# hukenovs/blackman_harris_win

Measured on AMD Instinct MI355X. Metric: window Gsamples/s (BH-7, N=2^26, 32-bit) + fraction of HBM-write roofline, higher is better.
Workload: dtype int64

## Files before the change

### blackman_harris_win_amd/csrc/bhw_build.hip

```cpp
#include "bhw_device.h"

namespace {

template <typename T>
__global__ __launch_bounds__(kBlock) void k_table_build(BhwCordicCfg cfg, uint32_t entries, void *__restrict__ table)
{
    __shared__ T lut_s[32];
    stage_lut<T>(cfg, lut_s);
    const uint32_t u = blockIdx.x * kBlock + threadIdx.x;
    if (u >= entries) return;
    T x, y;
    cordic_q1<T>(lut_s, (T)cfg.x0, (T)((T)u << cfg.z_shl), (int)cfg.n_iter, x, y);
    const int32_t c = (int32_t)(x >> cfg.out_shr), sn = (int32_t)(y >> cfg.out_shr);
    const int2 head = make_int2(__builtin_amdgcn_readfirstlane(c), __builtin_amdgcn_readfirstlane(sn));
    const int4 rec = cfg.tab_dlog > kPackLog ? reinterpret_cast<const int4 *>(cfg.tab_coarse)[u >> fmt_cell_log(cfg.tab_dlog)] : make_int4(0, 0, 0, 0);
    tab_store(table, u, cfg.phi_width - 2 - cfg.z_shr, cfg.tab_split, cfg.tab_dlog, const_cast<void *>(cfg.tab_coarse), c, sn, head, rec,
              cfg.tab_check);
}


template <int NITER, int FMT>
__global__ __launch_bounds__(kBuildThreads) void k_table_build_shared(BhwBuildPlan plan, void *__restrict__ table)
{
    __shared__ int64_t gx[kGroupsPerWg];
    __shared__ int64_t gy[kGroupsPerWg];
    __shared__ int32_t gz[kGroupsPerWg];
    __shared__ int32_t gk[kGroupsPerWg];
    __shared__ uint32_t lut_s[32];
    if (threadIdx.x < 32) lut_s[threadIdx.x] = plan.lut[threadIdx.x];
    __syncthreads();

    constexpr int n_iter = NITER;
    const uint32_t s = plan.z_shl;
    const uint32_t gpw = plan.groups_per_wg;
    const uint32_t group0 = blockIdx.x * gpw;
    const uint32_t n_groups = plan.entries >> 6;

    if (threadIdx.x < gpw) {
        const uint32_t g = group0 + threadIdx.x;
        const uint32_t u_first = g << 6;
        int64_t x = plan.x0, y = plan.x0;
        int32_t zf = (int32_t)((u_first << s) - lut_s[0]);
        const uint32_t span = 63u << s;
        int k = 1;
        bool live = g < n_groups;
        constexpr int kmax = n_iter < kPrefixMax ? n_iter : kPrefixMax;
#pragma unroll
        for (int kk = 1; kk < kmax; ++kk) {
            if (live) {
                const int32_t zl = (int32_t)((uint32_t)zf + span);
                if ((zf < 0) != (zl < 0)) {
                    live = false;
                } else {
                    rot_step(x, y, zf, kk, plan.lut[kk]);
                    k = kk + 1;
                }
            }
        }
        gx[threadIdx.x] = x;
        gy[threadIdx.x] = y;
        gz[threadIdx.x] = zf;
        gk[threadIdx.x] = k;
    }
    __syncthreads();

    const uint32_t wave = __builtin_amdgcn_readfirstlane(threadIdx.x >> 6), lane = threadIdx.x & 63u;
    uint32_t idx_a = lane, idx_m = 64u;
    if (plan.tab_split) {
        const uint32_t e = 1u << plan.log2_entries;
        if (lane & 1u)      { idx_a = (e >> 1) + (lane >> 1); idx_m = 32u; }
        else if (lane & 2u) { idx_a = (e >> 2) + (lane >> 2); idx_m = 16u; }
        else                { idx_a = lane >> 2;              idx_m = 16u; }
    }
    for (uint32_t gi = wave; gi < gpw; gi += kBuildThreads / 64) {
        const uint32_t g = __builtin_amdgcn_readfirstlane(group0 + gi);
        if (g >= n_groups) break;
        int64_t x = gx[gi], y = gy[gi];
        int32_t z = (int32_t)((uint32_t)gz[gi] + (lane << s));
        const int k0 = __builtin_amdgcn_readfirstlane(gk[gi]);
#pragma unroll
        for (int k = 1; k < NITER; ++k) {
            if (k >= kPrefixMax || k >= k0) rot_step(x, y, z, k, plan.lut[k]);
        }
        const int32_t c = (int32_t)(x >> plan.out_shr), sn = (int32_t)(y >> plan.out_shr);
        const int2 head = make_int2(__builtin_amdgcn_readfirstlane(c), __builtin_amdgcn_readfirstlane(sn));
        const uint32_t idx = idx_a + g * idx_m;
        if constexpr (FMT == 4) {
            const uint32_t u = (g << 6) + lane, nmask = 4u * plan.entries - 1u;
            int32_t *d_sin = reinterpret_cast<int32_t *>(table), *d_cos = reinterpret_cast<int32_t *>(const_cast<void *>(plan.tab_coarse));
#pragma unroll
            for (uint32_t q = 0; q < 4u; ++q) {
                int32_t oc, os;
                quadrant_map(q, c, sn, plan.pad0, oc, os);
                const uint32_t i = (q * plan.entries + u - plan.pad) & nmask;
                if (d_sin) d_sin[i] = os;
                if (d_cos) d_cos[i] = oc;
            }
        } else if constexpr (FMT == 0) {
            reinterpret_cast<int2 *>(table)[idx] = make_int2(c, sn);
        } else {
            static_assert(FMT == 1, "k_table_build_shared builds plain and delta16 tables (and the sin / cos sweep) only");
            const int32_t dc = c - head.x, ds = sn - head.y;
            if (plan.check_flag && !(fits_bits(dc, 16) && fits_bits(ds, 16))) atomicOr(plan.check_flag, 1u);
            reinterpret_cast<uint32_t *>(table)[idx] = ((uint32_t)dc & 0xFFFFu) | ((uint32_t)ds << 16);
            if (lane == 0u) reinterpret_cast<int2 *>(const_cast<void *>(plan.tab_coarse))[g] = head;
        }
    }
}

constexpr int kMirrorTail = 6;
constexpr int mirror_gpw(int threads) { return threads / 4; }
constexpr int mirror_heads_max(int threads) { return mirror_gpw(threads) / 2 + 8; }
constexpr int mirror_heads_pad(int threads) { return (mirror_heads_max(threads) + 63) / 64 * 64; }
constexpr int kTailZ = 256;

constexpr int kTailRows = 65;
struct TailD { int8_t v[kTailRows * 64 + 16]; };
constexpr TailD make_tail_d()
{
    TailD t{};
    for (int p = 0; p < 64; ++p)
        for (int v = 0; v < kTailRows; ++v) {
            int d = 0;
            for (int j = 0; j < kMirrorTail; ++j) d += ((p >> j) & 1) ? -(v >> j) : (v >> j);
            t.v[v * 64 + p] = (int8_t)d;
        }
    return t;
}
__device__ const TailD kTailD = make_tail_d();

template <int K, bool ZERO>
__device__ __forceinline__ void rot_narrow(uint32_t &x, uint32_t &y, int32_t &z, uint32_t &zacc, uint32_t lutk)
{
    uint32_t a, b;
    if constexpr (ZERO) {
        asm volatile("v_lshrrev_b32 %[a], %[k], %[y]\n\t"
                     "v_lshrrev_b32 %[b], %[k], %[x]\n\t"
                     "v_min_u32 %[za], %[za], %[z]\n\t"
                     "v_cmpx_gt_i32 vcc, 0, %[z]\n\t"
                     "v_add_u32 %[x], %[x], %[a]\n\t"
                     "v_sub_u32 %[y], %[y], %[b]\n\t"
                     "v_add_u32 %[z], %[z], %[l]\n\t"
                     "s_not_b64 exec, exec\n\t"
                     "v_sub_u32 %[x], %[x], %[a]\n\t"
                     "v_add_u32 %[y], %[y], %[b]\n\t"
                     "v_sub_u32 %[z], %[z], %[l]\n\t"
                     "s_mov_b64 exec, -1"
                     : [x] "+v"(x), [y] "+v"(y), [z] "+v"(z), [za] "+v"(zacc), [a] "=&v"(a), [b] "=&v"(b)
                     : [l] "s"(lutk), [k] "n"(K)
                     : "vcc", "scc");
    } else {
        asm volatile("v_lshrrev_b32 %[a], %[k], %[y]\n\t"
                     "v_lshrrev_b32 %[b], %[k], %[x]\n\t"
                     "v_cmpx_gt_i32 vcc, 0, %[z]\n\t"
                     "v_add_u32 %[x], %[x], %[a]\n\t"
                     "v_sub_u32 %[y], %[y], %[b]\n\t"
                     "v_add_u32 %[z], %[z], %[l]\n\t"
                     "s_not_b64 exec, exec\n\t"
                     "v_sub_u32 %[x], %[x], %[a]\n\t"
                     "v_add_u32 %[y], %[y], %[b]\n\t"
                     "v_sub_u32 %[z], %[z], %[l]\n\t"
                     "s_mov_b64 exec, -1"
                     : [x] "+v"(x), [y] "+v"(y), [z] "+v"(z), [a] "=&v"(a), [b] "=&v"(b)
                     : [l] "s"(lutk), [k] "n"(K)
                     : "vcc", "scc");
    }
}

template <int KA, int NITER>
__device__ __forceinline__ void rot_narrow_block(uint32_t &x, uint32_t &y, int32_t &z, uint32_t &zacc, const uint32_t *lut, int e, uint32_t hi)
{
    uint32_t a, b;
#define BHW_ROT_I(lbl, i, HI_ADD)                                                                                       \
    #lbl ":\n\t"                                                                                                        \
    "v_lshrrev_b32 %[a], %[k" #i "], %[y]\n\t"                                                                          \
    "v_lshrrev_b32 %[b], %[k" #i "], %[x]\n\t"                                                                          \
    HI_ADD                                                                                                             \
    "v_min_u32 %[za], %[za], %[z]\n\t"                                                                                  \
    "v_cmpx_gt_i32 vcc, 0, %[z]\n\t"                                                                                    \
    "v_add_u32 %[x], %[x], %[a]\n\t"                                                                                    \
    "v_sub_u32 %[y], %[y], %[b]\n\t"                                                                                    \
    "v_add_u32 %[z], %[z], %[l" #i "]\n\t"                                                                              \
    "s_not_b64 exec, exec\n\t"                                                                                          \
    "v_sub_u32 %[x], %[x], %[a]\n\t"                                                                                    \
    "v_add_u32 %[y], %[y], %[b]\n\t"                                                                                    \
    "v_sub_u32 %[z], %[z], %[l" #i "]\n\t"                                                                              \
    "s_mov_b64 exec, -1\n"
#define BHW_ROT_PLAIN(i) BHW_ROT_I(i, i, "")
#define BHW_ROT_HI(i) BHW_ROT_I(2##i, i, "v_add_u32 %[b], %[c" #i "], %[b]\n\t")
#define BHW_ROT_DISPATCH(P)                                                                                            \
                 "s_cmp_lt_i32 %[e], 1\n\ts_cbranch_scc1 " #P "0f\n\t"                                                 \
                 "s_cmp_eq_u32 %[e], 1\n\ts_cbranch_scc1 " #P "1f\n\t"                                                 \
                 "s_cmp_eq_u32 %[e], 2\n\ts_cbranch_scc1 " #P "2f\n\t"                                                 \
                 "s_cmp_eq_u32 %[e], 3\n\ts_cbranch_scc1 " #P "3f\n\t"                                                 \
                 "s_cmp_eq_u32 %[e], 4\n\ts_cbranch_scc1 " #P "4f\n\t"                                                 \
                 "s_cmp_eq_u32 %[e], 5\n\ts_cbranch_scc1 " #P "5f\n\t"                                                 \
                 "s_cmp_eq_u32 %[e], 6\n\ts_cbranch_scc1 " #P "6f\n\t"                                                 \
                 "s_cmp_eq_u32 %[e], 7\n\ts_cbranch_scc1 " #P "7f\n\t"                                                 \
                 "s_cmp_eq_u32 %[e], 8\n\ts_cbranch_scc1 " #P "8f\n\t"                                                 \
                 "s_cmp_eq_u32 %[e], 9\n\ts_cbranch_scc1 " #P "9f\n\t"
    constexpr int S = NITER - 1 - KA;
    static_assert(S >= 9 && S <= 30, "bias shifts");
    asm volatile("s_cmp_lg_u32 %[hi], 0\n\ts_cbranch_scc1 100f\n\t"
                 BHW_ROT_DISPATCH()
                 "s_branch 10f\n"
                 BHW_ROT_PLAIN(0) BHW_ROT_PLAIN(1) BHW_ROT_PLAIN(2) BHW_ROT_PLAIN(3) BHW_ROT_PLAIN(4) BHW_ROT_PLAIN(5) BHW_ROT_PLAIN(6) BHW_ROT_PLAIN(7)
                 BHW_ROT_PLAIN(8) BHW_ROT_PLAIN(9)
                 "10:\n\ts_branch 200f\n"
                 "100:\n\t"
                 BHW_ROT_DISPATCH(2)
                 "s_branch 200f\n"
                 BHW_ROT_HI(0) BHW_ROT_HI(1) BHW_ROT_HI(2) BHW_ROT_HI(3) BHW_ROT_HI(4) BHW_ROT_HI(5) BHW_ROT_HI(6) BHW_ROT_HI(7) BHW_ROT_HI(8) BHW_ROT_HI(9)
                 "200:"
                 : [x] "+v"(x), [y] "+v"(y), [z] "+v"(z), [za] "+v"(zacc), [a] "=&v"(a), [b] "=&v"(b)
                 : [e] "s"(e), [hi] "s"(hi), [l0] "s"(lut[KA]), [l1] "s"(lut[KA + 1]), [l2] "s"(lut[KA + 2]), [l3] "s"(lut[KA + 3]), [l4] "s"(lut[KA + 4]),
                   [l5] "s"(lut[KA + 5]), [l6] "s"(lut[KA + 6]), [l7] "s"(lut[KA + 7]), [l8] "s"(lut[KA + 8]), [l9] "s"(lut[KA + 9]),
                   [k0] "n"(KA), [k1] "n"(KA + 1), [k2] "n"(KA + 2), [k3] "n"(KA + 3), [k4] "n"(KA + 4), [k5] "n"(KA + 5), [k6] "n"(KA + 6),
                   [k7] "n"(KA + 7), [k8] "n"(KA + 8), [k9] "n"(KA + 9),
                   [c0] "n"(1 << S), [c1] "n"(1 << (S - 1)), [c2] "n"(1 << (S - 2)), [c3] "n"(1 << (S - 3)), [c4] "n"(1 << (S - 4)),
                   [c5] "n"(1 << (S - 5)), [c6] "n"(1 << (S - 6)), [c7] "n"(1 << (S - 7)), [c8] "n"(1 << (S - 8)), [c9] "n"(1 << (S - 9))
                 : "vcc", "scc");
#undef BHW_ROT_I
#undef BHW_ROT_PLAIN
#undef BHW_ROT_HI
#undef BHW_ROT_DISPATCH
}

#ifdef BHW_BUILD_STAMPS
__device__ unsigned long long *g_build_stamps = nullptr;
#define BHW_STAMP(i) do { if (g_build_stamps && (threadIdx.x & 63u) == 0u) atomicMax(&g_build_stamps[blockIdx.x * 16u + (i)], (unsigned long long)wall_clock64()); } while (0)
#define BHW_STAMP_MIN(i) do { if (g_build_stamps && threadIdx.x == 0u) g_build_stamps[blockIdx.x * 16u + (i)] = (unsigned long long)wall_clock64(); } while (0)
#else
#define BHW_STAMP(i) do { } while (0)
#define BHW_STAMP_MIN(i) do { } while (0)
#endif

template <int BYTES>
__device__ __forceinline__ void table_store(void *__restrict__ table, uint32_t idx, uint32_t v)
{
    if constexpr (BYTES == 1) asm volatile("global_store_byte %0, %1, %2 sc1" :: "v"(idx), "v"(v), "s"(table) : "memory");
    else asm volatile("global_store_short %0, %1, %2 sc1" :: "v"(idx << 1), "v"(v), "s"(table) : "memory");
}

template <int NITER, int FMT, int THREADS>
__global__ __launch_bounds__(THREADS) __attribute__((amdgpu_waves_per_eu(8, 8))) void k_table_build_mirror(BhwBuildPlan plan, void *__restrict__ table)
{
    BHW_STAMP_MIN(0);
#ifdef BHW_BUILD_STAMPS
    if (g_build_stamps && threadIdx.x == 0u) {
        uint32_t hw, xcc;
        asm volatile("s_getreg_b32 %0, hwreg(HW_REG_HW_ID)\n\ts_getreg_b32 %1, hwreg(HW_REG_XCC_ID)" : "=s"(hw), "=s"(xcc));
        g_build_stamps[blockIdx.x * 16u + 6u] = hw;
        g_build_stamps[blockIdx.x * 16u + 7u] = xcc;
    }
#endif
    static_assert(FMT == 2 || FMT == 3 || FMT == 5, "residual / nibble entries");
    static_assert(NITER >= 21 && NITER <= 32, "narrow state: 32-bit words");
    static_assert(THREADS == 256 || THREADS == 1024, "workgroup shapes");
    constexpr uint32_t gpw = mirror_gpw(THREADS);
    constexpr uint32_t kHeads = mirror_heads_max(THREADS), kHeadsPad = mirror_heads_pad(THREADS);
    static_assert(gpw + 2 * kHeadsPad + 64 <= THREADS, "prefix lanes, two ranges of head chains, the tail-table wave");
    __shared__ int64_t gx[gpw];
    __shared__ int64_t gy[gpw];
    __shared__ int32_t gz[gpw];
    __shared__ int32_t gk[gpw];
    __shared__ uint32_t gflag[gpw];
    __shared__ uint32_t lut_s[32];
    __shared__ uint8_t tail_p[2 * kTailZ];
    __shared__ __attribute__((aligned(16))) int8_t tail_d[kTailRows * 64 + 16];
    constexpr uint32_t kWorkMax = 8 * gpw;
    __shared__ uint32_t work_n;
    __shared__ uint32_t work_u[kWorkMax];
    __shared__ uint32_t esc_n;
    __shared__ int4 esc_list[FMT == 5 ? kEscFill : 1];
    __shared__ int4 esc_tab[FMT == 5 ? kEscSlots : 1];
    if (threadIdx.x < 32) lut_s[threadIdx.x] = plan.lut[threadIdx.x];
    if constexpr (FMT == 5) {
        if (threadIdx.x >= 64u && threadIdx.x < 64u + kEscSlots) esc_tab[threadIdx.x - 64u] = make_int4(-1, 0, 0, 0);
    }
#ifdef BHW_BUILD_STAMPS
    if (g_build_stamps && threadIdx.x == 0u) { asm volatile("s_waitcnt lgkmcnt(0)" ::: "memory"); g_build_stamps[blockIdx.x * 16u + 8u] = (unsigned long long)wall_clock64() | (plan.entries & 0u); }
#endif
    constexpr int n_iter = NITER;
    constexpr int KS = NITER - kMirrorTail;
    const uint32_t s = plan.z_shl;
    const uint32_t group0 = blockIdx.x * gpw;
    const uint32_t E = plan.entries;
    const uint32_t n_groups = E >> 7;
    const uint32_t u_lo = group0 << 6;
    const uint32_t u_hi = ((group0 + gpw) << 6) < (n_groups << 6) ? ((group0 + gpw) << 6) : (n_groups << 6);
    const uint32_t m_last = (E >> 1) - 1u;
    if (threadIdx.x == 0) {
        work_n = 0u;
        esc_n = 0u;
        if (u_hi == (E >> 1)) {
            work_u[0] = E >> 1;
            work_n = 1u;
        }
    }
    if (threadIdx.x >= (uint32_t)THREADS - 64u) {
        const uint32_t t3 = threadIdx.x - ((uint32_t)THREADS - 64u);
#pragma unroll
        for (int q = 0; q < 5; ++q)
            if (t3 + 64u * q < (uint32_t)(kTailRows * 64 + 16) / 16u) reinterpret_cast<int4 *>(tail_d)[t3 + 64u * q] = reinterpret_cast<const int4 *>(kTailD.v)[t3 + 64u * q];
#pragma unroll
        for (int q = 0; q < 2 * kTailZ / 64; ++q) {
            const uint32_t zi = t3 + 64u * (uint32_t)q;
            int32_t z = (int32_t)zi - kTailZ;
            uint32_t p = 0u;
#pragma unroll
            for (int j = 0; j < kMirrorTail; ++j) {
                if (z < 0) { p |= 1u << j; z += (int32_t)plan.lut[KS + j]; } else z -= (int32_t)plan.lut[KS + j];
            }
            tail_p[zi] = (uint8_t)p;
        }
        BHW_STAMP(9);
    }


    __shared__ int32_t hc[2][kHeads], hs[2][kHeads];
    const uint32_t d = fmt_cell_log(plan.tab_dlog);
    const uint32_t cells_total = E >> d;
    uint32_t cell_lo[2] = {0u, 0u}, n_cell[2] = {0u, 0u}, r_lo[2] = {u_lo, 0u}, r_hi[2] = {u_hi, 0u};
    {
        const uint32_t a = u_lo > 1u ? u_lo : 1u, b = (u_hi - 1u) < m_last ? (u_hi - 1u) : m_last;
        if (a <= b) { r_lo[1] = E - b; r_hi[1] = E - a + 1u; }
        if (a <= b && b == (E >> 1) - 1u) r_lo[1] = E >> 1;
    }
#pragma unroll
    for (int w = 0; w < 2; ++w)
        if (r_hi[w] > r_lo[w]) {
            cell_lo[w] = r_lo[w] >> d;
            n_cell[w] = ((r_hi[w] - 1u) >> d) - cell_lo[w] + 1u;
        }
    if (threadIdx.x >= gpw && threadIdx.x < gpw + 2u * kHeadsPad) {
        const uint32_t w = (threadIdx.x - gpw) / kHeadsPad;
        const uint32_t t = (threadIdx.x - gpw) % kHeadsPad;
        if (n_cell[w] && t < n_cell[w] + 2u) {
            const int64_t cell = (t <= n_cell[w]) ? (int64_t)cell_lo[w] + t : (int64_t)cell_lo[w] - 1;
            if (cell >= 0 && cell < (int64_t)cells_total) {
                int64_t x = plan.x0, y = plan.x0;
                int32_t z = (int32_t)((((uint32_t)cell << d) << s) - plan.lut[0]);
#pragma unroll
                for (int r = 1; r < n_iter; ++r) rot_step(x, y, z, r, plan.lut[r]);
                hc[w][t] = (int32_t)(x >> plan.out_shr);
                hs[w][t] = (int32_t)(y >> plan.out_shr);
            }
        }
        BHW_STAMP(10);
    }

    constexpr int kcap = KS < kPrefixMax ? KS : kPrefixMax;
    if (threadIdx.x < gpw) {
        const uint32_t g = group0 + threadIdx.x;
        const uint32_t u_first = g << 6;
        int64_t x = plan.x0, y = plan.x0;
        int32_t zf = (int32_t)((u_first << s) - plan.lut[0]);
        const uint32_t span = 63u << s;
        int k = 1;
        bool live = g < n_groups;
        uint32_t zero0 = 0u;
#pragma unroll
        for (int kk = 1; kk < kcap; ++kk) {
            if (live) {
                const int32_t zl = (int32_t)((uint32_t)zf + span);
                if ((zf < 0) != (zl < 0)) {
                    live = false;
                } else {
                    zero0 |= (uint32_t)(zf == 0);
                    rot_step(x, y, zf, kk, plan.lut[kk]);
                    k = kk + 1;
                }
            }
        }
        const int64_t drift = ((int64_t)1 << (NITER - k + 1)) + 2, lim = (int64_t)1 << NITER;
        const bool narrow = x >= drift && y >= drift && x + drift < lim && y + drift < lim;
        constexpr int64_t kBias = (int64_t)1 << (NITER - 1);
        const bool hi = !narrow && k >= KS - 10 && y >= drift && y + drift < lim && x - kBias >= drift && x - kBias + drift < ((int64_t)1 << 32) &&
                        x + drift < lim + ((int64_t)1 << KS);
        gx[threadIdx.x] = hi ? x - kBias : x;
        gy[threadIdx.x] = y;
        gz[threadIdx.x] = zf;
        gk[threadIdx.x] = k;
        gflag[threadIdx.x] = zero0 | (narrow || hi ? 2u : 0u) | (hi ? 4u : 0u);
        BHW_STAMP(11);
    }
    BHW_STAMP(1);
    __syncthreads();

    __shared__ int4 hrec[2][kHeads];
    {
        const uint32_t w = threadIdx.x / kHeadsPad, t = threadIdx.x % kHeadsPad;
        if (w < 2u && t < n_cell[w]) {
            const uint32_t cell = cell_lo[w] + t;
            int4 r;
            if (cell + 1u < cells_total) r = make_int4(hc[w][t], hs[w][t], hc[w][t + 1] - hc[w][t], hs[w][t + 1] - hs[w][t]);
            else {
                const uint32_t tp = t ? t - 1u : n_cell[w] + 1u;
                r = make_int4(hc[w][t], hs[w][t], hc[w][t] - hc[w][tp], hs[w][t] - hs[w][tp]);
            }
            if constexpr (FMT == 5) { r.x += (int32_t)kEscBias; r.y += (int32_t)kEscBias; }
            if constexpr (fmt_is_nibble(FMT)) { r.x -= 8; r.y -= 8; }
            hrec[w][t] = r;
            if constexpr (fmt_is_nibble(FMT)) { r.z *= 2; r.w *= 2; }
            if ((cell << d) >= r_lo[w])
                reinterpret_cast<int4 *>(const_cast<void *>(plan.tab_coarse))[cell] = r;
        }
    }
    __syncthreads();
    BHW_STAMP_MIN(2);
    auto record_of = [&](int w, uint32_t cell) -> int4 { return hrec[w][cell - cell_lo[w]]; };
    auto record = [&](int w, uint32_t cell) -> int4 {
        return record_of(w, __builtin_amdgcn_readfirstlane(cell));
    };

    auto store_entry = [&](uint32_t idx, int32_t c, int32_t sn, const int4 rec, uint32_t pos) {
        if constexpr (FMT == 5) {
            const int2 p = tab_predict(rec, pos, d);
            const uint32_t nc = (uint32_t)(c - p.x), ns = (uint32_t)(sn - p.y);
            uint32_t v = nc | (ns << 4);
            if (__builtin_expect((int)(nc - 1u > 14u) | (int)(ns > 15u), 0)) {
                const uint32_t slot = atomicAdd(&esc_n, 1u);
                if (slot < kEscFill) esc_list[slot] = make_int4((int32_t)idx, c, sn, 0);
                v = kEscMarker;
            }
            table_store<1>(table, idx, v);
        } else if constexpr (FMT == 3) {
            const int2 p = tab_predict(rec, pos, d);
            const uint32_t nc = (uint32_t)(c - p.x), ns = (uint32_t)(sn - p.y);
            if (plan.check_flag && (nc | ns) > 15u) atomicOr(plan.check_flag, 1u);
            table_store<1>(table, idx, nc | (ns << 4));
        } else {
            const int2 p = tab_predict(rec, pos, d);
            const int32_t dc = c - p.x, ds = sn - p.y;
            if (plan.check_flag && !(fits_bits(dc, 8) && fits_bits(ds, 8))) atomicOr(plan.check_flag, 1u);
            table_store<2>(table, idx, ((uint32_t)dc & 0xFFu) | ((uint32_t)ds << 8));
        }
    };

    const uint32_t wave = __builtin_amdgcn_readfirstlane(threadIdx.x >> 6), lane = threadIdx.x & 63u;
    uint32_t idx_a, idx_m, idx_i;
    if (lane & 1u)      { idx_a = (E >> 1) + (lane >> 1); idx_m = 32u; idx_i = E + (E >> 1) - 1u; }
    else if (lane & 2u) { idx_a = (E >> 2) + (lane >> 2); idx_m = 16u; idx_i = (E >> 1) + (E >> 2) - 1u; }
    else                { idx_a = lane >> 2;              idx_m = 16u; idx_i = E >> 2; }
    if (!plan.tab_split) { idx_a = lane; idx_m = 64u; idx_i = E; }
    const uint32_t fmask = (1u << d) - 1u;
    for (uint32_t gi = wave; gi < gpw; gi += THREADS / 64) {
        const uint32_t g = __builtin_amdgcn_readfirstlane(group0 + gi);
        if (g >= n_groups) break;
        {
            const uint32_t it = (gi - wave) / (uint32_t)(THREADS / 64);
            if (it == 0u) __builtin_amdgcn_s_setprio(3);
            else if (it == 4u) __builtin_amdgcn_s_setprio(2);
            else if (it == 8u) __builtin_amdgcn_s_setprio(1);
            else if (it == 12u) __builtin_amdgcn_s_setprio(0);
        }
        const int k0 = __builtin_amdgcn_readfirstlane(gk[gi]);
        const uint32_t gf = __builtin_amdgcn_readfirstlane(gflag[gi]);
        int32_t z = (int32_t)((uint32_t)gz[gi] + (lane << s));
        uint64_t zmask = 0ull;
        int32_t c1, s1, c2, s2;
        bool replay = false;
        if (gf & 2u) {
            uint32_t x = (uint32_t)gx[gi], y = (uint32_t)gy[gi];
            uint32_t zacc = ~0u;
            constexpr int KA = KS - 10;
            static_assert(KA >= 5 && KA < kcap && KS - KA == 10, "ten-rotation block");
            if (k0 < KA) {
#define BHW_NARROW(K) if constexpr (K < KA) { if (K >= k0) rot_narrow<K, true>(x, y, z, zacc, plan.lut[K]); }
                BHW_NARROW(1) BHW_NARROW(2) BHW_NARROW(3) BHW_NARROW(4) BHW_NARROW(5) BHW_NARROW(6) BHW_NARROW(7) BHW_NARROW(8)
                BHW_NARROW(9) BHW_NARROW(10) BHW_NARROW(11) BHW_NARROW(12) BHW_NARROW(13) BHW_NARROW(14) BHW_NARROW(15)
#undef BHW_NARROW
            }
            const bool hi = (gf & 4u) != 0u;
            rot_narrow_block<KA, NITER>(x, y, z, zacc, plan.lut, k0 - KA, hi ? 1u : 0u);
            zmask = __builtin_amdgcn_ballot_w64(zacc == 0u);
            const uint32_t xrow6 = hi ? (1u << (NITER - 1 - KS + 6)) : 0u;
            const uint32_t bias_out = hi ? ((1u << (NITER - 1)) >> plan.out_shr) : 0u;
            static_assert(KS <= 26, "unrolled to rotation 25");
            constexpr uint32_t lowm = (1u << KS) - 1u;
            const uint32_t zi = (uint32_t)(z + kTailZ);
            const uint32_t mx = (x + 128u) & lowm, my = (y + 128u) & lowm;
            const uint32_t unsafe = (uint32_t)((mx < my ? mx : my) < 256u) | (uint32_t)((zi - 1u) >= (uint32_t)(2 * kTailZ - 1));
            if (__builtin_amdgcn_ballot_w64(unsafe != 0u) == 0ull) {
                const uint32_t xx = ((x >> KS) << 6) + xrow6, yy = (y >> KS) << 6;
                const uint32_t p1 = tail_p[zi], p2 = tail_p[2u * kTailZ - zi];
                const int32_t dx1 = tail_d[p1 + yy], dy1 = tail_d[p1 + xx], dx2 = tail_d[p2 + xx], dy2 = tail_d[p2 + yy];
                c1 = (int32_t)(((x - (uint32_t)dx1) >> plan.out_shr) + bias_out);
                s1 = (int32_t)((y + (uint32_t)dy1) >> plan.out_shr);
                c2 = (int32_t)((y - (uint32_t)dx2) >> plan.out_shr);
                s2 = (int32_t)(((x + (uint32_t)dy2) >> plan.out_shr) + bias_out);
            } else if (hi) {
                int64_t xw = (int64_t)x + ((int64_t)1 << (NITER - 1)), yw = (int64_t)y;
                int64_t x2 = yw, y2 = xw;
                int32_t z2 = -z;
#pragma unroll 1
                for (int k = KS; k < NITER; ++k) {
                    rot_step_dyn(xw, yw, z, k, lut_s[k], true);
                    rot_step_dyn(x2, y2, z2, k, lut_s[k], true);
                }
                c1 = (int32_t)(xw >> plan.out_shr); s1 = (int32_t)(yw >> plan.out_shr);
                c2 = (int32_t)(x2 >> plan.out_shr); s2 = (int32_t)(y2 >> plan.out_shr);
            } else {
                uint32_t x2 = y, y2 = x;
                int32_t z2 = -z;
                uint32_t unused = 0u;
#define BHW_NARROW(K) if constexpr (K >= KS && K < NITER) { rot_narrow<K, false>(x, y, z, unused, plan.lut[K]); rot_narrow<K, false>(x2, y2, z2, unused, plan.lut[K]); }
                BHW_NARROW(15) BHW_NARROW(16) BHW_NARROW(17) BHW_NARROW(18) BHW_NARROW(19) BHW_NARROW(20) BHW_NARROW(21) BHW_NARROW(22)
                BHW_NARROW(23) BHW_NARROW(24) BHW_NARROW(25) BHW_NARROW(26) BHW_NARROW(27) BHW_NARROW(28) BHW_NARROW(29) BHW_NARROW(30)
                BHW_NARROW(31)
#undef BHW_NARROW
                c1 = (int32_t)(x >> plan.out_shr); s1 = (int32_t)(y >> plan.out_shr);
                c2 = (int32_t)(x2 >> plan.out_shr); s2 = (int32_t)(y2 >> plan.out_shr);
            }
        } else {
            int64_t x = gx[gi], y = gy[gi];
#pragma unroll 1
            for (int k = k0; k < KS; ++k) {
                zmask |= __builtin_amdgcn_ballot_w64(z == 0);
                rot_step_dyn(x, y, z, k, lut_s[k], k >= kMad24From);
            }
            int64_t x2 = y, y2 = x;
            int32_t z2 = -z;
#pragma unroll 1
            for (int k = KS; k < NITER; ++k) {
                rot_step_dyn(x, y, z, k, lut_s[k], true);
                rot_step_dyn(x2, y2, z2, k, lut_s[k], true);
            }
            c1 = (int32_t)(x >> plan.out_shr); s1 = (int32_t)(y >> plan.out_shr);
            c2 = (int32_t)(x2 >> plan.out_shr); s2 = (int32_t)(y2 >> plan.out_shr);
        }
        const uint32_t g6 = __builtin_amdgcn_readfirstlane(g << 6);
        const uint32_t u = g6 + lane;
        const bool has_image = u >= 1u && u <= m_last;
        bool deferred = false;
        if (zmask != 0ull || gf & 1u) {
            replay = has_image && ((((zmask >> lane) & 1ull) != 0ull) || ((gf & 1u) && lane == 0u));
            if (replay) {
                const uint32_t slot = atomicAdd(&work_n, 1u);
                if (slot < kWorkMax) { work_u[slot] = u; deferred = true; }
                else {
                    int64_t xf = plan.x0, yf = plan.x0;
                    int32_t zf = (int32_t)(((E - u) << s) - lut_s[0]);
#pragma unroll 1
                    for (int r = 1; r < n_iter; ++r) rot_step_dyn(xf, yf, zf, r, lut_s[r], r >= kMad24From);
                    c2 = (int32_t)(xf >> plan.out_shr);
                    s2 = (int32_t)(yf >> plan.out_shr);
                }
            }
        }
        const uint32_t idx = fmt_is_nibble(FMT) ? (g << 6) + lane : idx_a + g * idx_m;
        store_entry(idx, c1, s1, record(0, g6 >> d), (g6 & fmask) + lane);
        if (has_image && !deferred) {
            const uint32_t um = E - u;
            const uint32_t top = E - g6, cell_a = (top - 63u) >> d, cell_b = top >> d;
            const uint32_t cell_c = cell_a >= cell_lo[1] ? cell_a : cell_lo[1];
            int4 rec2 = record(1, cell_c);
            if (__builtin_amdgcn_readfirstlane(cell_b) != __builtin_amdgcn_readfirstlane(cell_c)) {
                const int4 rb = record(1, cell_b);
                if (lane == 0u) rec2 = rb;
            }
            store_entry(fmt_is_nibble(FMT) ? E - idx : idx_i - idx, c2, s2, rec2, um & fmask);
        }
    }
    BHW_STAMP_MIN(3);
    BHW_STAMP(4);
    __syncthreads();
    const uint32_t n_work = work_n < kWorkMax ? work_n : kWorkMax;
    for (uint32_t i = threadIdx.x; i < n_work; i += THREADS) {
        const uint32_t um = E - work_u[i];
        int64_t xf = plan.x0, yf = plan.x0;
        int32_t zf = (int32_t)((um << s) - plan.lut[0]);
#pragma unroll
        for (int r = 1; r < n_iter; ++r) rot_step(xf, yf, zf, r, plan.lut[r]);
        store_entry(tab_index(um, plan.log2_entries, plan.tab_split), (int32_t)(xf >> plan.out_shr), (int32_t)(yf >> plan.out_shr), record_of(1, um >> d), um & fmask);
    }
    if constexpr (FMT == 5) {
        __syncthreads();
        const uint32_t n_esc = esc_n < kEscFill ? esc_n : kEscFill;
        uint32_t tid = threadIdx.x;
        asm volatile("" : "+v"(tid));
        if (tid < n_esc) {
            const int4 it = esc_list[tid];
            uint32_t h = esc_slot((uint32_t)it.x);
#pragma unroll 1
            for (uint32_t i = 0; i < kEscSlots; ++i) {
                const uint32_t was = atomicCAS(reinterpret_cast<uint32_t *>(&esc_tab[h].x), ~0u, (uint32_t)it.x);
                if (was == ~0u || was == (uint32_t)it.x) { esc_tab[h].y = it.y; esc_tab[h].z = it.z; break; }
                h = (h + 1u) & (kEscSlots - 1u);
            }
        }
        __syncthreads();
        if (tid < kEscSlots) reinterpret_cast<int4 *>(plan.tab_esc)[(size_t)blockIdx.x * kEscSlots + tid] = esc_tab[tid];
        if (tid == 0u && esc_n > kEscFill && plan.check_flag) atomicOr(plan.check_flag, 1u);
    }
    BHW_STAMP(5);
}

template <int NITER>
__global__ __launch_bounds__(kBlock) void k_table_build_plain(BhwCordicCfg cfg, uint32_t entries, int2 *__restrict__ table)
{
    __shared__ uint32_t lut_s[32];
    if (threadIdx.x < 32) lut_s[threadIdx.x] = (uint32_t)cfg.lut[threadIdx.x];
    __syncthreads();
    const uint32_t u = blockIdx.x * kBlock + threadIdx.x;
    if (u >= entries) return;
    int64_t x = cfg.x0, y = cfg.x0;
    int32_t z = (int32_t)((u << cfg.z_shl) - lut_s[0]);
#pragma unroll
    for (int r = 1; r < NITER; ++r) rot_step(x, y, z, r, lut_s[r]);
    table[u] = make_int2((int32_t)(x >> cfg.out_shr), (int32_t)(y >> cfg.out_shr));
}

}


int bhwk_sincos_sweep(const BhwLaunch &l, const BhwCordicCfg &c, uint64_t theta0, int32_t *d_sin, int32_t *d_cos)
{
    hipStream_t st = (hipStream_t)l.stream;
    BhwBuildPlan plan;
    for (uint32_t k = 0; k < 32; ++k) plan.lut[k] = (uint32_t)c.lut[k];
    plan.entries = 1u << (c.phi_width - 2);
    plan.n_iter = c.n_iter;
    plan.z_shl = c.z_shl;
    plan.out_shr = c.out_shr;
    plan.log2_entries = c.phi_width - 2;
    plan.tab_split = 0;
    plan.tab_dlog = 0;
    plan.pad0 = c.ones_neg;
    plan.tab_coarse = d_cos;
    plan.x0 = c.x0;
    plan.check_flag = nullptr;
    plan.tab_esc = nullptr;
    const unsigned groups = plan.entries >> 6;
    plan.groups_per_wg = groups >= 64u * 1024u ? 64u : groups >= 16u * 1024u ? 16u : 4u;
    plan.pad = (uint32_t)(theta0 & ((1ull << c.phi_width) - 1ull));
    const dim3 grid((groups + plan.groups_per_wg - 1) / plan.groups_per_wg), block(kBuildThreads);
    if (!with_int_range<7, 32>(c.n_iter, [&](auto N) { launch(k_table_build_shared<N, 4>, grid, block, st, plan, (void *)d_sin); }))
        return (int)hipErrorInvalidValue;
    return finish(hipSuccess);
}

#ifdef BHW_BUILD_STAMPS
extern "C" int bhw_dbg_build_stamps(void *d_words)
{
    unsigned long long *p = (unsigned long long *)d_words;
    return (int)hipMemcpyToSymbol(HIP_SYMBOL(g_build_stamps), &p, sizeof p);
}
#endif

int bhwk_table_build(const BhwLaunch &l, const BhwCordicCfg &c_in, int32_t *d_table)
{
    const BhwCordicCfg c = table_layout(c_in);
    hipStream_t st = (hipStream_t)l.stream;
    const uint32_t entries = 1u << (c.phi_width - 2 - c.z_shr);
    const bool fits = (c.dat_width + c.out_shr <= 34);
    if (fits && c.n_iter >= 7 && entries < (1u << 20) && c.tab_dlog == 0 && !c.tab_split) {
        const dim3 grid(grid_for(entries)), block(kBlock);
        if (!with_int_range<7, 32>(c.n_iter, [&](auto N) { launch(k_table_build_plain<N>, grid, block, st, c, entries, (int2 *)d_table); }))
            return (int)hipErrorInvalidValue;
        return finish(hipSuccess);
    }
    if (entries >= 64 && fits && c.n_iter >= 2) {
        BhwBuildPlan plan;
        for (uint32_t k = 0; k < 32; ++k) plan.lut[k] = (uint32_t)c.lut[k];
        plan.entries = entries;
        plan.n_iter = c.n_iter;
        plan.z_shl = c.z_shl;
        plan.out_shr = c.out_shr;
        plan.log2_entries = c.phi_width - 2 - c.z_shr;
        plan.tab_split = c.tab_split;
        plan.tab_dlog = c.tab_dlog;
        plan.pad0 = 0;
        plan.tab_coarse = c.tab_coarse;
        plan.x0 = c.x0;
        plan.check_flag = c.tab_check;
        plan.tab_esc = const_cast<void *>(c.tab_esc);
        const unsigned groups = entries >> 6;
        plan.groups_per_wg = groups >= 64u * 1024u ? 64u : groups >= 16u * 1024u ? 16u : 4u;
        plan.pad = 0;
        const dim3 grid((groups + plan.groups_per_wg - 1) / plan.groups_per_wg), block(kBuildThreads);
        const int fmt = fmt_of(c.tab_dlog);
        if (c.n_iter < 21 && fmt != 0) return (int)hipErrorInvalidValue;
        if (bhwk_build_mirror_applies(c, entries)) {
            const unsigned own_groups = entries >> 7;
            const unsigned threads = bhwk_build_mirror_threads(entries);
            const unsigned mgpw = (unsigned)mirror_gpw((int)threads);
            const dim3 mgrid((own_groups + mgpw - 1) / mgpw), mblock(threads);
            plan.groups_per_wg = mgpw;
            const bool listed = with_int_range<21, 32>(c.n_iter, [&](auto N) {
                with_int_or_last<2, 3, 5>(fmt, [&](auto F) {
                    with_int_or_last<1024, 256>((int)threads, [&](auto T) {
                        launch(k_table_build_mirror<N, F, T>, mgrid, mblock, st, plan, (void *)d_table);
                    });
                });
            });
            return listed ? finish(hipSuccess) : (int)hipErrorInvalidValue;
        }
        if (fmt > 1) return (int)hipErrorInvalidValue;
        const bool listed = with_int_range<7, 32>(c.n_iter, [&](auto N) {
            if constexpr (N < 21) launch(k_table_build_shared<N, 0>, grid, block, st, plan, (void *)d_table);
            else with_int_or_last<0, 1>(fmt, [&](auto F) { launch(k_table_build_shared<N, F>, grid, block, st, plan, (void *)d_table); });
        });
        return listed ? finish(hipSuccess) : (int)hipErrorInvalidValue;
    }
    if (c.tab_dlog > kPackLog) return (int)hipErrorInvalidValue;
    if (c.wide) launch(k_table_build<int64_t>, dim3(grid_for(entries)), dim3(kBlock), st, c, entries, (void *)d_table);
    else        launch(k_table_build<int32_t>, dim3(grid_for(entries)), dim3(kBlock), st, c, entries, (void *)d_table);
    return finish(hipSuccess);
}
```

Measured before the change: 703.5.

## Build coarse records via wave shuffles and make prefix CORDIC branchless

When both coarse-cell windows fit in one wavefront, head-record deltas are now computed with __shfl from neighbouring lanes and written directly. This skips the shared hc/hs round trip and one __syncthreads barrier. The group prefix CORDIC loop is split into a branchless angle pass, which tracks sign masks, liveness and a zero flag, followed by a rotation pass driven by those masks. This is meant to remove divergent branching. The cost is more ALU work in the rotation pass, and the shuffle indexing assumes the head lanes t<64 share one wavefront, with src masked to 63.

```diff
diff --git a/blackman_harris_win_amd/csrc/bhw_build.hip b/blackman_harris_win_amd/csrc/bhw_build.hip
--- a/blackman_harris_win_amd/csrc/bhw_build.hip
+++ b/blackman_harris_win_amd/csrc/bhw_build.hip
@@ -333,45 +333,79 @@
             cell_lo[w] = r_lo[w] >> d;
             n_cell[w] = ((r_hi[w] - 1u) >> d) - cell_lo[w] + 1u;
         }
+    __shared__ int4 hrec[2][kHeads];
+    auto put_record = [&](uint32_t w, uint32_t t, uint32_t cell, uint32_t first, int32_t c, int32_t sn, int32_t dc, int32_t ds) {
+        int4 r = make_int4(c, sn, dc, ds);
+        if constexpr (FMT == 5) { r.x += (int32_t)kEscBias; r.y += (int32_t)kEscBias; }
+        if constexpr (fmt_is_nibble(FMT)) { r.x -= 8; r.y -= 8; }
+        hrec[w][t] = r;
+        if constexpr (fmt_is_nibble(FMT)) { r.z *= 2; r.w *= 2; }
+        if ((cell << d) >= first)
+            reinterpret_cast<int4 *>(const_cast<void *>(plan.tab_coarse))[cell] = r;
+    };
+    const bool rec_early = n_cell[0] + 2u <= 64u && n_cell[1] + 2u <= 64u;
     if (threadIdx.x >= gpw && threadIdx.x < gpw + 2u * kHeadsPad) {
         const uint32_t w = (threadIdx.x - gpw) / kHeadsPad;
         const uint32_t t = (threadIdx.x - gpw) % kHeadsPad;
-        if (n_cell[w] && t < n_cell[w] + 2u) {
-            const int64_t cell = (t <= n_cell[w]) ? (int64_t)cell_lo[w] + t : (int64_t)cell_lo[w] - 1;
+        const uint32_t ncw = w ? n_cell[1] : n_cell[0], clw = w ? cell_lo[1] : cell_lo[0];
+        int32_t c = 0, sn = 0;
+        if (ncw && t < ncw + 2u) {
+            const int64_t cell = (t <= ncw) ? (int64_t)clw + t : (int64_t)clw - 1;
             if (cell >= 0 && cell < (int64_t)cells_total) {
                 int64_t x = plan.x0, y = plan.x0;
                 int32_t z = (int32_t)((((uint32_t)cell << d) << s) - plan.lut[0]);
 #pragma unroll
                 for (int r = 1; r < n_iter; ++r) rot_step(x, y, z, r, plan.lut[r]);
-                hc[w][t] = (int32_t)(x >> plan.out_shr);
-                hs[w][t] = (int32_t)(y >> plan.out_shr);
+                c = (int32_t)(x >> plan.out_shr);
+                sn = (int32_t)(y >> plan.out_shr);
+                if (!rec_early) { hc[w][t] = c; hs[w][t] = sn; }
             }
         }
         BHW_STAMP(10);
+        if (rec_early && t < 64u) {
+            const bool last = clw + t + 1u >= cells_total;
+            const uint32_t src = (last ? (t ? t - 1u : ncw + 1u) : t + 1u) & 63u;
+            const int32_t nc = __shfl(c, (int)src), ns = __shfl(sn, (int)src);
+            if (t < ncw) put_record(w, t, clw + t, w ? r_lo[1] : r_lo[0], c, sn, last ? c - nc : nc - c, last ? sn - ns : ns - sn);
+            BHW_STAMP(12);
+        }
     }
 
     constexpr int kcap = KS < kPrefixMax ? KS : kPrefixMax;
     if (threadIdx.x < gpw) {
         const uint32_t g = group0 + threadIdx.x;
         const uint32_t u_first = g << 6;
-        int64_t x = plan.x0, y = plan.x0;
         int32_t zf = (int32_t)((u_first << s) - plan.lut[0]);
         const uint32_t span = 63u << s;
         int k = 1;
-        bool live = g < n_groups;
-        uint32_t zero0 = 0u;
+        int32_t sticky = g < n_groups ? 0 : INT32_MIN;
+        uint32_t zacc = ~0u;
+        uint32_t negm = 0u;
+        int32_t zw = zf;
 #pragma unroll
         for (int kk = 1; kk < kcap; ++kk) {
-            if (live) {
-                const int32_t zl = (int32_t)((uint32_t)zf + span);
-                if ((zf < 0) != (zl < 0)) {
-                    live = false;
-                } else {
-                    zero0 |= (uint32_t)(zf == 0);
-                    rot_step(x, y, zf, kk, plan.lut[kk]);
-                    k = kk + 1;
-                }
-            }
+            const int32_t m = zw >> 31;
+            sticky |= zw ^ (int32_t)((uint32_t)zw + span);
+            const int32_t dead = sticky >> 31;
+            negm |= (uint32_t)m & (1u << kk);
+            const uint32_t zz = (uint32_t)zw | (uint32_t)dead;
+            zacc = zz < zacc ? zz : zacc;
+            zw = (int32_t)((uint32_t)zw - plan.lut[kk] + 2u * ((uint32_t)m & plan.lut[kk]));
+            zf = (int32_t)(((uint32_t)zf & (uint32_t)dead) | ((uint32_t)zw & ~(uint32_t)dead));
+            k += 1 + dead;
+            asm volatile("" : "+v"(k), "+v"(zf), "+v"(zacc));
+        }
+        const uint32_t zero0 = zacc == 0u ? 1u : 0u;
+        const uint32_t act = (1u << k) - 2u, fwdm = ~negm & act, bwdm = negm & act;
+        int64_t x = plan.x0, y = plan.x0;
+#pragma unroll
+        for (int kk = 1; kk < kcap; ++kk) {
+            const int32_t nsg = ((int32_t)(fwdm << (31 - kk)) >> 31) - ((int32_t)(bwdm << (31 - kk)) >> 31);
+            int32_t ys = (int32_t)(y >> kk);
+            int32_t xs = (int32_t)(x >> kk);
+            asm volatile("" : "+v"(ys), "+v"(xs));
+            x += (int64_t)nsg * (int64_t)ys;
+            y += (int64_t)(-nsg) * (int64_t)xs;
         }
         const int64_t drift = ((int64_t)1 << (NITER - k + 1)) + 2, lim = (int64_t)1 << NITER;
         const bool narrow = x >= drift && y >= drift && x + drift < lim && y + drift < lim;
@@ -388,26 +422,20 @@
     BHW_STAMP(1);
     __syncthreads();
 
-    __shared__ int4 hrec[2][kHeads];
-    {
+    if (!rec_early) {
         const uint32_t w = threadIdx.x / kHeadsPad, t = threadIdx.x % kHeadsPad;
-        if (w < 2u && t < n_cell[w]) {
-            const uint32_t cell = cell_lo[w] + t;
-            int4 r;
-            if (cell + 1u < cells_total) r = make_int4(hc[w][t], hs[w][t], hc[w][t + 1] - hc[w][t], hs[w][t + 1] - hs[w][t]);
+        const uint32_t ncw = w ? n_cell[1] : n_cell[0], first = w ? r_lo[1] : r_lo[0];
+        if (w < 2u && t < ncw) {
+            const int32_t c = hc[w][t], sn = hs[w][t];
+            const uint32_t cell = (w ? cell_lo[1] : cell_lo[0]) + t;
+            if (cell + 1u < cells_total) put_record(w, t, cell, first, c, sn, hc[w][t + 1] - c, hs[w][t + 1] - sn);
             else {
-                const uint32_t tp = t ? t - 1u : n_cell[w] + 1u;
-                r = make_int4(hc[w][t], hs[w][t], hc[w][t] - hc[w][tp], hs[w][t] - hs[w][tp]);
-            }
-            if constexpr (FMT == 5) { r.x += (int32_t)kEscBias; r.y += (int32_t)kEscBias; }
-            if constexpr (fmt_is_nibble(FMT)) { r.x -= 8; r.y -= 8; }
-            hrec[w][t] = r;
-            if constexpr (fmt_is_nibble(FMT)) { r.z *= 2; r.w *= 2; }
-            if ((cell << d) >= r_lo[w])
-                reinterpret_cast<int4 *>(const_cast<void *>(plan.tab_coarse))[cell] = r;
-        }
-    }
-    __syncthreads();
+                const uint32_t tp = t ? t - 1u : ncw + 1u;
+                put_record(w, t, cell, first, c, sn, c - hc[w][tp], sn - hs[w][tp]);
+            }
+        }
+        __syncthreads();
+    }
     BHW_STAMP_MIN(2);
     auto record_of = [&](int w, uint32_t cell) -> int4 { return hrec[w][cell - cell_lo[w]]; };
     auto record = [&](int w, uint32_t cell) -> int4 {
```

Result: no change. 701.4 (median of 2 runs) (-0.3%).
